# tamask1s/rspt

Hardware: AMD Instinct MI355X
Metric: MSamples/s compress (xdelta_hzr, 64ch x 65536 int32) (higher is better)
Workload: dtype int32

## Files before the change

rspt_amd/csrc/common.hpp:

```cpp
#pragma once
#include <hip/hip_runtime.h>
#include <stdint.h>

#ifdef RSPT_DIAG
#define RSPT_DIAG_ONLY(x) (x)
#else
#define RSPT_DIAG_ONLY(x) 0u
#endif

namespace rspt {

constexpr uint32_t kHzrBlock = 65536;
constexpr int kNumSym = 261;
constexpr uint32_t kRunCap = 16662;
constexpr int kSymStride = 264;
constexpr int kTdescWords = 92;
constexpr int kWave = 64;
constexpr int kEncThreads = 1024;
constexpr int kEncWaves = kEncThreads / kWave;
constexpr int kMaxPlanes = 4;
constexpr uint32_t kKindBytes = 4;

enum : uint32_t { kModeCopy = 0, kModeHuff = 1, kModeFill = 2, kModeSkip = 3, kModeStaged = 4 };

constexpr uint32_t kStageSlotWords = 772;

struct Geom {
    uint32_t bps, nch, ns;
    uint32_t N;
    uint32_t nblk;
    uint32_t hdr_len;
    uint32_t method;
    uint32_t kind;
    uint32_t be;
    uint64_t plane_stride;
// ... 240 lines not shown
```

rspt_amd/csrc/host_budget.hip:

```cpp
static size_t budget_tab_bytes(size_t nblocks, size_t nladder) { return (nladder * nblocks * sizeof(uint64_t) + 255) & ~(size_t)255; }

static bool budget_batched_ok(const rspt_hip_packer* p, size_t nblocks, size_t nladder) {
    const Geom& g = p->g;
    return g.kind == RSPT_HIP_KIND_HADAMARD && g.ns <= kTpMaxNs && nladder * nblocks <= 65535;
}

static int budget_route(const rspt_hip_packer* p, size_t nblocks, size_t nladder) {
    const bool ok = budget_batched_ok(p, nblocks, nladder);
    if (p->budget_route == 2) return ok ? 1 : RSPT_HIP_ERR_UNSUPPORTED;
    return p->budget_route == 0 && ok ? 1 : 0;
}

int rspt_hip_debug_set_budget_route(rspt_hip_packer* p, int route) {
    if (!p || route < 0 || route > 2) return RSPT_HIP_ERR_ARG;
    if (route == 2 && !budget_batched_ok(p, 1, 1)) return RSPT_HIP_ERR_UNSUPPORTED;
    p->budget_route = (uint32_t)route;
    return RSPT_HIP_OK;
}

int rspt_hip_compress_budget_work_bytes(rspt_hip_packer* p, size_t nblocks, size_t nladder, size_t* bytes) {
    if (!bytes) return RSPT_HIP_ERR_ARG;
    if (int rc = target_checks(p, nblocks, nladder)) return rc;
    if (int r = budget_route(p, nblocks, nladder); r < 0) return r;
    *bytes = budget_tab_bytes(nblocks, nladder);
// ... 24 lines not shown
}

static int budget_sizes_batched(rspt_hip_packer* p, const void* d_src, size_t nblocks, const LadderSel& ls, unsigned long long* tab,
                                hipStream_t st) {
    const Geom& g = p->g;
    const uint32_t B = (uint32_t)nblocks, S = ls.fwd.n * B;
    if (int rc = rspt_hip_reserve(p, S)) return rc;
    if (int rc = front_begin(p, S, st)) return rc;
    int32_t* orig = p->ws.planar + (size_t)(S - B) * g.N;
    if (int rc = rspt_hip_native_to_i32_batch_dev(p, d_src, orig, nblocks, (void*)st)) return rc;
    const uint32_t nt = std::max(64u, std::min(1024u, g.ns / kTpPer));
    const uint32_t lds = tp_pad(g.ns) * (uint32_t)sizeof(uint32_t);
    hipLaunchKernelGGL(k_budget_probe, dim3(g.nch, B), dim3(nt), lds, st, (const int32_t*)orig, g, ls.fwd, B, (int32_t*)p->ws.planar);
    hipLaunchKernelGGL((k_planar_planes<false>), dim3((g.N + 4095) / 4096, S), dim3(256), 0, st, p->ws.planar, g, (uint32_t)p->nb_host, p->ws.planes,
                       p->nzflag, (uint32_t*)nullptr);
    hipLaunchKernelGGL(k_nb_scan, dim3(1), dim3(1024), 0, st, p->needmask, S, p->nb_state, p->ws.nbuse, 0);
    const uint32_t nhb = S * kMaxPlanes * g.nblk;
    hipLaunchKernelGGL(k_histlist, dim3((nhb + 255) / 256), dim3(256), 0, st, p->nzflag, p->ws.nbuse, g, nhb, p->ws.big_list, p->work_ctr + 2, p->psel);
    HIPCHK(p, hipGetLastError());
    if (int rc = phase_hist(p, S, st)) return rc;
    if (int rc = phase_tree(p, S, st)) return rc;
    return budget_pass_end(p, S, tab, st);
}

int rspt_hip_compress_budget_batch_dev(rspt_hip_packer* p, const void* d_src, size_t nblocks, const double* ladder, size_t nladder,
                                       size_t budget_bytes, const uint64_t* d_budget, void* d_dst, size_t dst_stride, uint64_t* d_sizes,
                                       uint32_t* d_choice, uint64_t* d_cand_sizes, void* d_work, void* stream) {
    static_assert(sizeof(size_t) == sizeof(uint64_t), "budget_bytes carries any uint64");
    if (!p || !d_src || !d_dst || !d_sizes || !d_choice || !d_work || nblocks == 0) return RSPT_HIP_ERR_ARG;
    if ((reinterpret_cast<uintptr_t>(d_src) & 15) || (reinterpret_cast<uintptr_t>(d_choice) & 3) || (reinterpret_cast<uintptr_t>(d_budget) & 7) ||
        (reinterpret_cast<uintptr_t>(d_cand_sizes) & 7) || (reinterpret_cast<uintptr_t>(d_work) & 15))
        return RSPT_HIP_ERR_ARG;
    if (p->feed) return RSPT_HIP_ERR_ARG;
// ... 18 lines not shown
```

rspt_amd/csrc/host_handle.hpp:

```cpp
#pragma once

namespace {
enum Stage { ST_PRE = 0, ST_NB, ST_HIST, ST_TREE, ST_LAYOUT, ST_ENCODE, ST_COUNT };
const char* kStageNames[ST_COUNT] = {"preprocess", "nb_scan", "hzr_hist", "hzr_tree", "layout", "hzr_encode"};
}

template <class T, auto Release>
class Owned {
  public:
    Owned() = default;
    Owned(Owned&& o) noexcept : h_(o.h_) { o.h_ = nullptr; }
    Owned& operator=(Owned&& o) noexcept {
        if (this != &o) {
            reset();
            h_ = o.h_;
            o.h_ = nullptr;
        }
        return *this;
    }
    ~Owned() { reset(); }
    void reset() {
        if (h_) Release(h_);
        h_ = nullptr;
    }
// ... 7 lines not shown
    T h_ = nullptr;
};
template <class T> using Dev = Owned<T*, hipFree>;
template <class T> using Pinned = Owned<T*, hipHostFree>;
using Event = Owned<hipEvent_t, hipEventDestroy>;
using Stream = Owned<hipStream_t, hipStreamDestroy>;

struct Workspace {
    size_t cap_blocks = 0;
    size_t cap_slots = 0;
    Dev<uint8_t> planes;
    Dev<int32_t> planar;
    Dev<uint32_t> nbuse;
    Dev<uint32_t> dec_nb;
    Dev<uint32_t> big_list;
    Dev<uint32_t> staging;
    Dev<uint32_t> zbuf[2];
    size_t zcap_words = 0;
    bool zero_ready[2] = {false, false};
    int zset = 0;
    Dev<uint32_t> plane_dirty;
    bool planes_unknown = false;
    Dev<uint32_t> hist;
    Dev<uint32_t> seghist;
    Dev<uint32_t> segbase;
    Dev<uint32_t> lists;
    Dev<uint2> listinfo;
    Dev<uint32_t> cw;
    Dev<uint32_t> tdesc;
    Dev<BlockMeta> meta;
// ... 139 lines not shown
    double had_div_fwd = 0, had_div_inv = 0;
    bool dct_fft = false;
    uint32_t fft_l1 = 0, fft_l2 = 0;
    bool dct_real = false;
    uint32_t fftr_la = 0, fftr_lb = 0;
    uint32_t ntile = 0;
    uint32_t Tn_native = 0;
    uint32_t T = 0, in_lds = 0;
    uint32_t Tp[5] = {0, 0, 0, 0, 0};
    bool wide = false;
    uint32_t k1_threads = 256;
    uint32_t k1_grid = 0;
    uint32_t hist_grid = 0;
    uint32_t enc_grid = 0;
    uint32_t ablate = 0;
    uint32_t psel = 0;
    uint32_t target_route = 0;
    uint32_t budget_route = 0;
    uint32_t qp_form = 0;
    int verify = 0;
    int big_endian = 0;
    bool profiling = false;
    bool ev_valid = false;
    bool conv_lds_raised = false;

    Stream stream;
    Event ev[ST_COUNT + 1];
    Dev<unsigned long long> stamps;
    Dev<CrcConsts> crc;
    Dev<uint32_t> nb_state;
// ... 48 lines not shown
```

rspt_amd/csrc/hzr_kernels.hip:

```cpp
#include "common.hpp"

namespace rspt {

__device__ __forceinline__ uint32_t thread_id() {
    uint32_t t = threadIdx.x;
    asm volatile("" : "+v"(t));
    return t;
}

__device__ __forceinline__ uint32_t granule_byte_dyn(uint32_t w0, uint32_t w1, uint32_t w2, uint32_t w3, uint32_t i) {
    const uint32_t lo = (i & 8u) ? w2 : w0, hi = (i & 8u) ? w3 : w1;
    return __builtin_amdgcn_perm(hi, lo, 0x0C0C0C00u | (i & 7u));
}

constexpr uint32_t kWipeTokens = 2048;
__device__ __forceinline__ bool block_is_wiped(const BlockMeta& m) {
    return m.mode == kModeStaged || (m.mode == kModeHuff && m.fill <= kWipeTokens);
}
constexpr uint32_t kSmallSegments = 2;
constexpr uint32_t kSmallTokens = 512;
constexpr uint32_t kSmallPayload = 3072;
static_assert(kStageSlotWords * 4 >= 7 + kSmallPayload + 4 + 4, "staging slot too small");

struct WorkQueues {
    uint32_t n_big;
    uint32_t next_big;
};

struct WorkItem {
    uint32_t b, k, j;
};
__device__ __forceinline__ bool next_work(uint32_t* counter, uint32_t total, const Geom& g, uint32_t* s_slot, WorkItem& wi, uint32_t pass) {
    __syncthreads();
    if (threadIdx.x == 0) *s_slot = pass == 0 ? blockIdx.x : gridDim.x + atomicAdd(counter, 1u);
// ... 941 lines not shown
```

rspt_amd/csrc/planar.hip:

```cpp
#include "common.hpp"

namespace rspt {

constexpr uint32_t kPlanarThreads = 256;

__device__ __forceinline__ uint32_t cut_to_width(uint32_t v, uint32_t sx) { return (uint32_t)((int32_t)(v << sx) >> sx); }

template <bool XDELTA>
__global__ __launch_bounds__(kPlanarThreads) void k_planar_stream(const int32_t* __restrict__ src, Geom g, uint32_t kfirst, uint32_t kcount,
                                                                 uint8_t* __restrict__ planes, uint32_t* __restrict__ needmask,
                                                                 uint32_t* __restrict__ nzflag, const uint32_t* __restrict__ nbuse, uint32_t nblocks,
                                                                 uint32_t* __restrict__ ticket, uint32_t* __restrict__ nb_state,
                                                                 uint32_t* __restrict__ nbuse_out, const uint32_t* __restrict__ plane_dirty,
                                                                 uint32_t dirty_shift) {
    const uint32_t tid = threadIdx.x, l = lane_id();
    const bool fixup = nbuse != nullptr;
    if (fixup && *nb_state <= kfirst) return;
    const uint32_t sx = 32u - 8u * g.bps;
    const uint32_t segs = (g.N + 4095u) >> 12;
    const uint64_t total = (uint64_t)nblocks * segs;
    const uint64_t per = (total + gridDim.x - 1) / gridDim.x;
    const uint64_t w0 = (uint64_t)blockIdx.x * per, w1 = w0 + per < total ? w0 + per : total;
    uint32_t sent_b = 0xFFFFFFFFu, sent_f = 0;
    for (uint64_t w = w0; w < w1; ++w) {
        const uint32_t b = (uint32_t)(w / segs), seg = (uint32_t)(w - (uint64_t)b * segs);
        if (fixup && nbuse[b] <= kfirst) continue;
        const uint32_t off = (seg << 12) + tid * 16u;
        const uint32_t cnt = off < g.N ? min(16u, g.N - off) : 0u;
        const int32_t* pb = src + (size_t)b * g.N;
// ... 69 lines not shown
            if ((f & ~sent_f) && l == 0) atomicOr(&needmask[b], f);
            sent_f |= f;
        }
    }
    if (ticket) {
        __shared__ uint32_t s_last, s_wmax[16];
        __syncthreads();
        if (tid == 0) {
            __threadfence();
            s_last = atomicAdd(ticket, 1u) == gridDim.x - 1 ? 1u : 0u;
        }
        __syncthreads();
        if (s_last) {
            __threadfence();
            nb_scan_body(needmask, nblocks, nb_state, nbuse_out, XDELTA ? 1 : 0, s_wmax);
        }
    }
}
template __global__ void k_planar_stream<true>(const int32_t*, Geom, uint32_t, uint32_t, uint8_t*, uint32_t*, uint32_t*, const uint32_t*, uint32_t, uint32_t*, uint32_t*, uint32_t*, const uint32_t*, uint32_t);
template __global__ void k_planar_stream<false>(const int32_t*, Geom, uint32_t, uint32_t, uint8_t*, uint32_t*, uint32_t*, const uint32_t*, uint32_t, uint32_t*, uint32_t*, uint32_t*, const uint32_t*, uint32_t);

__global__ __launch_bounds__(256) void k_planar_ingest(const int32_t* __restrict__ src, Geom g, int32_t* __restrict__ planar,
                                                      long long* __restrict__ row_sum) {
    const uint32_t c = blockIdx.y, b = blockIdx.z, tid = threadIdx.x;
    const uint32_t sx = 32u - 8u * g.bps;
    const size_t base = (size_t)b * g.N + (size_t)c * g.ns;
    const uint32_t t0 = blockIdx.x * 4096u, t1 = min(g.ns, t0 + 4096u);
    long long sm = 0;
    for (uint32_t t = t0 + tid; t < t1; t += 256u) {
        const int32_t v = (int32_t)cut_to_width((uint32_t)src[base + t], sx);
        planar[base + t] = v;
        sm += v;
    }
    if (row_sum) {
#pragma unroll
// ... 20 lines not shown
```

rspt_amd/csrc/preprocess.hip:

```cpp
#include "common.hpp"

namespace rspt {

__device__ __forceinline__ uint32_t magic_of(uint32_t d) { return (uint32_t)(((1ull << 32) + d - 1) / d); }
__device__ __forceinline__ uint32_t fast_div(uint32_t q, uint32_t d, uint32_t M) { return d == 1 ? q : __umulhi(q, M); }

template <int BPS>
__device__ __forceinline__ int32_t sample_from_bytes(const uint8_t* p, bool aligned, bool be = false) {
    if (be) {
        if (BPS == 4) {
            if (aligned) {
                const uint32_t u = *reinterpret_cast<const uint32_t*>(p);
                return (int32_t)__builtin_amdgcn_perm(u, u, 0x00010203u);
            }
            return (int32_t)((uint32_t)p[3] | ((uint32_t)p[2] << 8) | ((uint32_t)p[1] << 16) | ((uint32_t)p[0] << 24));
        } else if (BPS == 3) {
            const uint32_t u = (uint32_t)p[2] | ((uint32_t)p[1] << 8) | ((uint32_t)p[0] << 16);
            return (int32_t)(u << 8) >> 8;
        } else if (BPS == 2) {
            const uint32_t u = (uint32_t)p[1] | ((uint32_t)p[0] << 8);
            return (int32_t)(u << 16) >> 16;
        }
        return (int32_t)(int8_t)p[0];
    }
// ... 35 lines not shown
    for (uint32_t b = lo; b < hi; ++b) m = max(m, need(b));
    const uint32_t l = lane_id(), w = tid >> 6;
    const uint32_t v = wave_scan_incl(m, 0u, [](uint32_t a, uint32_t c) { return a > c ? a : c; });
    if (l == 63) wmax[w] = v;
    __syncthreads();
    uint32_t pre = carry_in;
    for (uint32_t i = 0; i < w; ++i) pre = max(pre, wmax[i]);
    const uint32_t excl = dpp<0x138>(0u, v);
    uint32_t run = max(pre, l ? excl : 0u);
    for (uint32_t b = lo; b < hi; ++b) {
        run = max(run, need(b));
        nbuse[b] = run;
    }
    __syncthreads();
    if (tid == nthr - 1) *nb_state = max(pre, v);
}

struct ItemRegs {
    uint32_t pv[16];
    uint32_t p1, p2;
};

template <int BPS, bool XDELTA>
__device__ __forceinline__ void load_item(const uint8_t* blk, const Geom& g, uint32_t m_nch, uint32_t s0, uint32_t Tn, bool aligned4,
                                          uint32_t q, ItemRegs& R) {
    const size_t rstride = (size_t)g.nch * BPS;
    const uint32_t grp = fast_div(q, g.nch, m_nch);
    const uint32_t c = q - grp * g.nch;
    const uint32_t t0 = grp << 4;
    const uint32_t cnt = min(16u, Tn - t0);
// ... 131 lines not shown
#pragma unroll
            for (uint32_t k = 0; k < 4; ++k) {
                if (!((need >> k) & 1u)) continue;
                if (!(atomicOr(&za[k * g.nch], ba) & ba)) atomicOr(&nzflag[hb_index(g, b, k, ja)], ba);
                if (two && !(atomicOr(&zz[k * g.nch], bz) & bz)) atomicOr(&nzflag[hb_index(g, b, k, jz)], bz);
            }
        }
    }
}

template <int BPS, bool XDELTA>
__global__ __launch_bounds__(1024) void k_tile_planes(const uint8_t* __restrict__ src, Geom g, uint32_t T, uint32_t kfirst, uint32_t kcount,
                                                     uint8_t* __restrict__ planes, uint32_t* __restrict__ needmask,
                                                     uint32_t* __restrict__ nzflag, const uint32_t* __restrict__ nbuse, uint32_t ablate,
                                                     uint32_t nblocks, uint32_t* __restrict__ ticket, uint32_t* __restrict__ nb_state,
                                                     uint32_t* __restrict__ nbuse_out) {
    extern __shared__ __attribute__((aligned(16))) uint8_t lds[];
    const uint32_t tid = threadIdx.x, nthr = blockDim.x;
    const bool fixup = nbuse != nullptr;
    if (fixup && *nb_state <= kfirst) return;
    const uint32_t tiles_per_block = (g.ns + T - 1) / T;
    const uint32_t total = tiles_per_block * nblocks;
    const uint32_t m_nch = magic_of(g.nch);
    auto skip_untouched = [&](uint32_t wk) {
        while (wk < total && fixup && nbuse[wk / tiles_per_block] <= kfirst) wk += gridDim.x;
        return wk;
    };
    auto tile_s0 = [&](uint32_t wk) { return (wk - (wk / tiles_per_block) * tiles_per_block) * T; };
    uint32_t work = skip_untouched(blockIdx.x);
    ItemRegs cur, nxt, nx2;
    if (work < total) {
        const uint32_t s0f = tile_s0(work), Tnf = min(T, g.ns - s0f);
        const uint8_t* blkf = src + (size_t)(work / tiles_per_block) * g.block_bytes;
        if (tid < g.nch * ((Tnf + 15) >> 4))
// ... 69 lines not shown
        }
    }
    work = work_next;
    }
    if (ticket) {
        __shared__ uint32_t s_last, s_wmax[16];
        __syncthreads();
        if (tid == 0) {
            __threadfence();
            s_last = atomicAdd(ticket, 1u) == gridDim.x - 1 ? 1u : 0u;
        }
        __syncthreads();
        if (s_last) {
            __threadfence();
            nb_scan_body(needmask, nblocks, nb_state, nbuse_out, XDELTA ? 1 : 0, s_wmax);
        }
    }
}

template <int BPS>
__device__ __forceinline__ uint32_t stream_load(const uint8_t* base, uint32_t off) {
    uint32_t v;
    if (BPS == 1)
        asm volatile("global_load_sbyte %0, %1, %2" : "=v"(v) : "v"(off), "s"(base));
    else if (BPS == 2)
        asm volatile("global_load_sshort %0, %1, %2" : "=v"(v) : "v"(off), "s"(base));
    else
        asm volatile("global_load_dword %0, %1, %2" : "=v"(v) : "v"(off), "s"(base));
    return v;
}
// ... 501 lines not shown
        const uint32_t qpr = Tn >> 2;
        const uint32_t step_c = 256u / qpr, step_t = 256u - step_c * qpr;
        uint32_t c = tid / qpr, t4 = tid - c * qpr;
        for (uint32_t u = tid; u < g.nch * qpr; u += 256) {
            const int32_t* r = tile + c * RS + 4u * t4;
            *reinterpret_cast<int4*>(planar + (size_t)b * g.N + (size_t)c * g.ns + s0 + 4u * t4) = make_int4(r[0], r[1], r[2], r[3]);
            t4 += step_t;
            const uint32_t carry = t4 >= qpr ? 1u : 0u;
            t4 -= carry ? qpr : 0u;
            c += step_c + carry;
        }
    }
}

__global__ __launch_bounds__(1024) void k_nb_scan(const uint32_t* __restrict__ needmask, uint32_t nblocks, uint32_t* __restrict__ nb_state,
                                                  uint32_t* __restrict__ nbuse, int use_mask) {
    __shared__ uint32_t wmax[16];
    nb_scan_body(needmask, nblocks, nb_state, nbuse, use_mask, wmax);
}

#define INST_TILE(BPS)                                                                                                   \
    template __global__ void k_tile_planes<BPS, true>(const uint8_t*, Geom, uint32_t, uint32_t, uint32_t, uint8_t*, uint32_t*, uint32_t*, const uint32_t*, uint32_t, uint32_t, uint32_t*, uint32_t*, uint32_t*);    \
    template __global__ void k_tile_planes<BPS, false>(const uint8_t*, Geom, uint32_t, uint32_t, uint32_t, uint8_t*, uint32_t*, uint32_t*, const uint32_t*, uint32_t, uint32_t, uint32_t*, uint32_t*, uint32_t*);   \
    template __global__ void k_tile_planar<BPS>(const uint8_t*, Geom, uint32_t, int32_t*);
INST_TILE(1)
INST_TILE(2)
INST_TILE(3)
INST_TILE(4)
template __global__ void k_tile_stream<1, true, false>(const uint8_t*, Geom, uint32_t, uint32_t, uint32_t, uint8_t*, uint32_t*, uint32_t*, const uint32_t*, uint32_t, uint32_t, uint32_t*, uint32_t*, uint32_t*, const uint32_t*, uint32_t);
template __global__ void k_tile_stream<1, true, true>(const uint8_t*, Geom, uint32_t, uint32_t, uint32_t, uint8_t*, uint32_t*, uint32_t*, const uint32_t*, uint32_t, uint32_t, uint32_t*, uint32_t*, uint32_t*, const uint32_t*, uint32_t);
template __global__ void k_tile_stream<1, false, false>(const uint8_t*, Geom, uint32_t, uint32_t, uint32_t, uint8_t*, uint32_t*, uint32_t*, const uint32_t*, uint32_t, uint32_t, uint32_t*, uint32_t*, uint32_t*, const uint32_t*, uint32_t);
template __global__ void k_tile_stream<1, false, true>(const uint8_t*, Geom, uint32_t, uint32_t, uint32_t, uint8_t*, uint32_t*, uint32_t*, const uint32_t*, uint32_t, uint32_t, uint32_t*, uint32_t*, uint32_t*, const uint32_t*, uint32_t);
template __global__ void k_tile_stream<2, true, false>(const uint8_t*, Geom, uint32_t, uint32_t, uint32_t, uint8_t*, uint32_t*, uint32_t*, const uint32_t*, uint32_t, uint32_t, uint32_t*, uint32_t*, uint32_t*, const uint32_t*, uint32_t);
template __global__ void k_tile_stream<3, true, false>(const uint8_t*, Geom, uint32_t, uint32_t, uint32_t, uint8_t*, uint32_t*, uint32_t*, const uint32_t*, uint32_t, uint32_t, uint32_t*, uint32_t*, uint32_t*, const uint32_t*, uint32_t);
template __global__ void k_tile_stream<4, true, false>(const uint8_t*, Geom, uint32_t, uint32_t, uint32_t, uint8_t*, uint32_t*, uint32_t*, const uint32_t*, uint32_t, uint32_t, uint32_t*, uint32_t*, uint32_t*, const uint32_t*, uint32_t);
template __global__ void k_tile_stream<2, true, true>(const uint8_t*, Geom, uint32_t, uint32_t, uint32_t, uint8_t*, uint32_t*, uint32_t*, const uint32_t*, uint32_t, uint32_t, uint32_t*, uint32_t*, uint32_t*, const uint32_t*, uint32_t);
template __global__ void k_tile_stream<3, true, true>(const uint8_t*, Geom, uint32_t, uint32_t, uint32_t, uint8_t*, uint32_t*, uint32_t*, const uint32_t*, uint32_t, uint32_t, uint32_t*, uint32_t*, uint32_t*, const uint32_t*, uint32_t);
template __global__ void k_tile_stream<4, true, true>(const uint8_t*, Geom, uint32_t, uint32_t, uint32_t, uint8_t*, uint32_t*, uint32_t*, const uint32_t*, uint32_t, uint32_t, uint32_t*, uint32_t*, uint32_t*, const uint32_t*, uint32_t);
// ... 11 lines not shown
```

rspt_amd/csrc/rspt_hip.hip:

```cpp
#include "../../include/rspt_hip.h"

#include <hip/hip_runtime.h>
#include <dlfcn.h>
#include <link.h>
#include <climits>
#include <string>

#include <cmath>
#include <cstdio>
#include <cstdlib>
#include <cstring>
#include <memory>
#include <new>
#include <thread>
#include <type_traits>
#include <utility>
#include <vector>

#include "common.hpp"

#include "preprocess.hip"
#include "hzr_kernels.hip"
#include "hzr_rows.hip"
#include "transforms.hip"
// ... 94 lines not shown
    return T4 > g.ns ? g.ns : T4;
}

template <int BPS, bool XD>
static void launch_planes(rspt_hip_packer* p, const uint8_t* d_src, size_t nblocks, uint32_t kfirst, uint32_t kcount, const uint32_t* nbuse,
                          hipStream_t st) {
    const Geom& g = p->g;
    const uint32_t T = p->Tp[kcount];
    const bool stream_ok = (reinterpret_cast<uintptr_t>(d_src) & 3u) == 0 && g.ns >= 16 && g.block_bytes < (1ull << 32) && !(p->ablate & (1u << 22));
    const uint32_t lds = kcount * g.nch * (T + 16u) + 32u * g.nch + 96u;
    const uint32_t ntiles = (uint32_t)((g.ns + T - 1) / T * nblocks);
    const uint32_t per_cu = lds <= 40 * 1024 ? 4u : lds <= 80 * 1024 ? 2u : 1u;
    uint32_t want = per_cu * (uint32_t)p->num_cu;
    if (p->k1_grid) want = p->k1_grid;
    dim3 grid(want < ntiles ? want : ntiles);
    const bool stream = stream_ok;
    if (stream) {
        constexpr int SB = BPS;
        auto go = [&](auto kern) {
            hipFuncSetAttribute(reinterpret_cast<const void*>(kern), hipFuncAttributeMaxDynamicSharedMemorySize, (int)lds);
            hipLaunchKernelGGL(kern, grid, dim3(256), lds, st, d_src, g, T, kfirst, kcount, p->ws.planes, p->needmask, p->nzflag, nbuse, p->ablate,
                               (uint32_t)nblocks, nbuse ? nullptr : p->work_ctr + 1, p->nb_state, p->ws.nbuse, p->ws.plane_dirty, p->dirty_shift);
        };
        if (g.ns & 15u)
            go(&k_tile_stream<SB, XD, true>);
        else
            go(&k_tile_stream<SB, XD, false>);
        return;
    }
    hipFuncSetAttribute(reinterpret_cast<const void*>(&k_tile_planes<BPS, XD>), hipFuncAttributeMaxDynamicSharedMemorySize, (int)lds);
    hipLaunchKernelGGL((k_tile_planes<BPS, XD>), grid, dim3(p->k1_threads), lds, st, d_src, g, T, kfirst, kcount, p->ws.planes, p->needmask, p->nzflag, nbuse, p->ablate, (uint32_t)nblocks,
                       nbuse ? nullptr : p->work_ctr + 1, p->nb_state, p->ws.nbuse);
}

template <int BPS>
static uint32_t launch_front(rspt_hip_packer* p, const uint8_t* d_src, size_t nblocks, hipStream_t st) {
    const Geom& g = p->g;
    if (p->wide) {
        hipLaunchKernelGGL(k_wide_planar<BPS>, dim3((g.ns + 63) / 64, (g.nch + 63) / 64, (unsigned)nblocks), dim3(256), 0, st, d_src, g, p->ws.planar);
        if (g.kind == RSPT_HIP_KIND_XDELTA_HZR || g.kind == RSPT_HIP_KIND_HZR) {
            const bool xd = g.kind == RSPT_HIP_KIND_XDELTA_HZR;
            const dim3 pg((g.N + 4095) / 4096, (unsigned)nblocks);
            if (xd)
                hipLaunchKernelGGL((k_planar_planes<true>), pg, dim3(256), 0, st, p->ws.planar, g, 4u, p->ws.planes, p->nzflag, p->needmask);
            else
                hipLaunchKernelGGL((k_planar_planes<false>), pg, dim3(256), 0, st, p->ws.planar, g, 4u, p->ws.planes, p->nzflag, (uint32_t*)nullptr);
            hipLaunchKernelGGL(k_nb_scan, dim3(1), dim3(1024), 0, st, p->needmask, (uint32_t)nblocks, p->nb_state, p->ws.nbuse, xd ? 1 : 0);
        }
        return 4;
    }
    if (g.kind == RSPT_HIP_KIND_XDELTA_HZR) {
        const uint32_t np = p->nb_host;
        launch_planes<BPS, true>(p, d_src, nblocks, 0, np, nullptr, st);
        return np;
    }
    if (g.kind == RSPT_HIP_KIND_HZR) {
        launch_planes<BPS, false>(p, d_src, nblocks, 0, 4, nullptr, st);
        return 4;
    }
    if (BPS == 4 && (g.nch & 3) == 0 && (g.ns & 3) == 0 && g.nch <= 1024 && (reinterpret_cast<uintptr_t>(d_src) & 15) == 0) {
        const uint32_t T4 = tile_i32x4(g);
        hipLaunchKernelGGL(k_tile_planar_i32x4, dim3((g.ns + T4 - 1) / T4, (unsigned)nblocks), dim3(256), g.nch * (T4 + 1) * 4, st, d_src, g, T4,
// ... 3 lines not shown
    }
    dim3 grid((g.ns + p->T - 1) / p->T, (unsigned)nblocks);
    hipFuncSetAttribute(reinterpret_cast<const void*>(&k_tile_planar<BPS>), hipFuncAttributeMaxDynamicSharedMemorySize, (int)p->in_lds);
    hipLaunchKernelGGL((k_tile_planar<BPS>), grid, dim3(256), p->in_lds, st, d_src, g, p->T, p->ws.planar);
    return 4;
}

template <bool XD>
static void launch_planar_stream(rspt_hip_packer* p, const int32_t* d_planar, size_t nblocks, uint32_t kfirst, uint32_t kcount, const uint32_t* nbuse,
                                 hipStream_t st) {
    const Geom& g = p->g;
    const uint64_t units = (uint64_t)nblocks * ((g.N + 4095u) >> 12);
    const uint64_t want = 8ull * (uint64_t)p->num_cu;
    hipLaunchKernelGGL(k_planar_stream<XD>, dim3((uint32_t)(units < want ? units : want)), dim3(kPlanarThreads), 0, st, d_planar, g, kfirst, kcount, p->ws.planes,
                       p->needmask, p->nzflag, nbuse, (uint32_t)nblocks, nbuse ? nullptr : p->work_ctr + 1, p->nb_state, p->ws.nbuse, p->ws.plane_dirty,
                       p->dirty_shift);
}

static uint32_t launch_front_planar(rspt_hip_packer* p, const int32_t* d_planar, size_t nblocks, hipStream_t st) {
    const Geom& g = p->g;
    if (g.kind == RSPT_HIP_KIND_XDELTA_HZR) {
        const uint32_t np = p->nb_host;
        launch_planar_stream<true>(p, d_planar, nblocks, 0, np, nullptr, st);
        return np;
    }
    if (g.kind == RSPT_HIP_KIND_HZR) {
        launch_planar_stream<false>(p, d_planar, nblocks, 0, 4, nullptr, st);
        return 4;
    }
    hipLaunchKernelGGL(k_planar_ingest, dim3((g.ns + 4095u) / 4096u, g.nch, (unsigned)nblocks), dim3(256), 0, st, d_planar, g, p->ws.planar, p->row_sum);
    p->have_row_sum = p->row_sum != nullptr;
// ... 404 lines not shown
    HIPCHK(p, hipStreamSynchronize(p->stream));
    p->ws = Workspace();
    const Geom& g = p->g;
    Workspace w;
    const bool bare = g.kind == RSPT_HIP_KIND_BYTES;
    const size_t slots = slots_of(p, max_blocks);
    const size_t nhb = slots * kMaxPlanes * g.nblk;
    bool ok = true;
    ok &= hipMalloc(w.planes.out(), slots * kMaxPlanes * g.plane_stride + 4096) == hipSuccess;
    ok &= hipMalloc(w.nbuse.out(), max_blocks * sizeof(uint32_t)) == hipSuccess;
    ok &= hipMalloc(w.dec_nb.out(), max_blocks * sizeof(uint32_t)) == hipSuccess;
    ok &= hipMalloc(w.plane_dirty.out(), slots * kMaxPlanes * 4 * sizeof(uint32_t)) == hipSuccess;
    w.zcap_words = nhb + max_blocks + 32 + 2 * max_blocks * (size_t)g.nch + 2;
    for (int i = 0; i < 2; ++i) ok &= hipMalloc(w.zbuf[i].out(), w.zcap_words * sizeof(uint32_t)) == hipSuccess;
    ok &= hipMalloc(w.big_list.out(), nhb * sizeof(uint32_t)) == hipSuccess;
    ok &= hipMalloc(w.staging.out(), nhb * (size_t)kStageSlotWords * sizeof(uint32_t)) == hipSuccess;
    ok &= hipMalloc(w.hist.out(), nhb * kSymStride * sizeof(uint32_t)) == hipSuccess;
    ok &= hipMalloc(w.cw.out(), nhb * kSymStride * sizeof(uint32_t)) == hipSuccess;
    ok &= hipMalloc(w.seghist.out(), nhb * (size_t)kSegHistStride * sizeof(uint16_t)) == hipSuccess;
    ok &= hipMalloc(w.segbase.out(), nhb * (size_t)kEncWaves * sizeof(uint32_t)) == hipSuccess;
    ok &= hipMalloc(w.lists.out(), nhb * (size_t)kEncWaves * kListCap * sizeof(uint32_t)) == hipSuccess;
    ok &= hipMalloc(w.listinfo.out(), nhb * (size_t)kEncWaves * sizeof(uint2)) == hipSuccess;
    ok &= hipMalloc(w.tdesc.out(), nhb * kTdescWords * sizeof(uint32_t)) == hipSuccess;
    ok &= hipMalloc(w.meta.out(), nhb * sizeof(BlockMeta)) == hipSuccess;
    ok &= hipMalloc(w.out_off.out(), nhb * sizeof(uint64_t)) == hipSuccess;
    ok &= hipMalloc(w.means.out(), max_blocks * (size_t)(g.hdr_len ? g.hdr_len : 4)) == hipSuccess;
    if (!bare) ok &= hipMalloc(w.planar.out(), max_blocks * (size_t)g.N * sizeof(int32_t) + 4096) == hipSuccess;
    const size_t nscan = std::max<size_t>(p->ntile, g.N / kRowTile + 1);
    if (!bare) ok &= hipMalloc(w.txor.out(), max_blocks * nscan * sizeof(uint32_t)) == hipSuccess;
    if (!bare) ok &= hipMalloc(w.tsum.out(), max_blocks * nscan * sizeof(uint32_t)) == hipSuccess;
// ... 77 lines not shown
                               p->cos_tab, p->dct_scale0, p->dct_scale1, p->dct_cs0, p->ws.planar2);
        }
        hipLaunchKernelGGL((k_planar_planes<true>), dim3((g.N + 4095) / 4096, B), dim3(256), 0, st, p->ws.planar2, g, lossy_nb, p->ws.planes, nzflag, (uint32_t*)nullptr);
    }
}

static int front_begin(rspt_hip_packer* p, size_t nblocks, hipStream_t st) {
    const Geom& g = p->g;
    const size_t nhb_call = slots_of(p, nblocks) * kMaxPlanes * g.nblk;
    p->nzflag = p->ws.zbuf[p->ws.zset];
    p->needmask = p->nzflag + nhb_call;
    p->work_ctr = p->needmask + ((nblocks + 3) & ~(size_t)3);
    size_t zwords = (size_t)((p->work_ctr + 16) - p->nzflag);
    p->row_sum = nullptr;
    p->have_row_sum = false;
    if (g.kind == RSPT_HIP_KIND_DCT && p->dct_fft) {
        zwords = (zwords + 1) & ~(size_t)1;
        p->row_sum = reinterpret_cast<long long*>(p->nzflag + zwords);
        zwords += 2 * nblocks * (size_t)g.nch;
    }
    if (!p->ws.zero_ready[p->ws.zset]) HIPCHK(p, hipMemsetAsync(p->nzflag, 0, zwords * sizeof(uint32_t), st));
    p->ws.zero_ready[0] = p->ws.zero_ready[1] = false;
    if (p->ws.planes_unknown || (p->ablate & ~(3u << 26)) || p->psel) {
        HIPCHK(p, hipMemsetAsync(p->ws.plane_dirty, 0xFF, p->ws.cap_slots * kMaxPlanes * 4 * sizeof(uint32_t), st));
        p->ws.planes_unknown = false;
    }
    return RSPT_HIP_OK;
}

static int phase_front(rspt_hip_packer* p, const uint8_t* src, size_t nblocks, hipStream_t st, const int32_t* d_planar = nullptr, const LadderSel* ls = nullptr) {
    const Geom& g = p->g;
    const uint32_t B = (uint32_t)nblocks;
    stamp(p, ST_PRE, st);
    const bool xd = g.kind == RSPT_HIP_KIND_XDELTA_HZR;
    if (int rc = front_begin(p, nblocks, st)) return rc;
    if (g.kind == RSPT_HIP_KIND_BYTES) {
        const uint64_t units = (uint64_t)nblocks * ((g.N + 4095u) >> 12);
        const uint64_t want = 8ull * (uint64_t)p->num_cu;
        hipLaunchKernelGGL(k_bytes_ingest, dim3((uint32_t)(units < want ? units : want)), dim3(kIngestThreads), 0, st, src, g, B, p->ws.planes, p->nzflag,
                           p->ws.nbuse, p->ws.plane_dirty, p->dirty_shift);
        HIPCHK(p, hipGetLastError());
        stamp(p, ST_NB, st);
        stamp(p, ST_HIST, st);
        const uint32_t nhb = (uint32_t)slots_of(p, nblocks) * kMaxPlanes * g.nblk;
        hipLaunchKernelGGL(k_histlist, dim3((nhb + 255) / 256), dim3(256), 0, st, p->nzflag, p->ws.nbuse, g, nhb, p->ws.big_list, p->work_ctr + 2, p->psel);
        HIPCHK(p, hipGetLastError());
        return RSPT_HIP_OK;
    }
    const uint32_t np = d_planar ? launch_front_planar(p, d_planar, nblocks, st)
                                 : by_bps(g.bps, [&](auto bps) { return launch_front<decltype(bps)::value>(p, src, nblocks, st); });
    launch_forward_transform(p, B, st, p->nzflag, ls);
    HIPCHK(p, hipGetLastError());

    stamp(p, ST_NB, st);
    if (g.kind != RSPT_HIP_KIND_XDELTA_HZR && g.kind != RSPT_HIP_KIND_HZR)
        hipLaunchKernelGGL(k_nb_scan, dim3(1), dim3(1024), 0, st, p->needmask, B, p->nb_state, p->ws.nbuse, 0);
    if (xd && np < 4) {
        if (d_planar)
            launch_planar_stream<true>(p, d_planar, nblocks, np, 4 - np, p->ws.nbuse, st);
        else
            by_bps(g.bps, [&](auto bps) { launch_fixup<decltype(bps)::value>(p, src, nblocks, np, st); });
    }
    stamp(p, ST_HIST, st);
    const uint32_t nhb = B * kMaxPlanes * g.nblk;
    hipLaunchKernelGGL(k_histlist, dim3((nhb + 255) / 256), dim3(256), 0, st, p->nzflag, p->ws.nbuse, g, nhb, p->ws.big_list, p->work_ctr + 2, p->psel);
    HIPCHK(p, hipGetLastError());
    return RSPT_HIP_OK;
}

static uint32_t persistent_grid(const rspt_hip_packer* p, uint32_t nhb, uint32_t knob) {
    const uint32_t persist = (uint32_t)(2 * p->num_cu) < nhb ? (uint32_t)(2 * p->num_cu) : nhb;
    return knob && knob < persist ? knob : persist;
}

static int phase_hist(rspt_hip_packer* p, uint32_t B, hipStream_t st) {
    const Geom& g = p->g;
    const uint32_t nhb = B * kMaxPlanes * g.nblk;
    hipLaunchKernelGGL(k_hist, dim3(persistent_grid(p, nhb, p->hist_grid)), dim3(kEncThreads), 0, st, p->ws.planes, g, p->nzflag, p->ws.hist, p->ws.seghist, p->work_ctr,
                       p->ws.big_list, p->work_ctr + 2, p->ws.lists, p->ws.listinfo);
    HIPCHK(p, hipGetLastError());
    return RSPT_HIP_OK;
}

static int phase_tree(rspt_hip_packer* p, uint32_t B, hipStream_t st) {
    const Geom& g = p->g;
    const uint32_t nhb = B * kMaxPlanes * g.nblk;
    hipLaunchKernelGGL(k_tree, dim3((nhb + 3) / 4), dim3(256), 0, st, p->ws.hist, p->ws.planes, g, p->ws.nbuse, p->nzflag, nhb, p->ws.cw, p->ws.tdesc, p->ws.meta, p->ws.seghist, p->ws.segbase,
                       p->ws.zbuf[p->ws.zset ^ 1], (uint32_t)p->ws.zcap_words, p->crc, p->ws.staging, p->psel);
    HIPCHK(p, hipGetLastError());
    return RSPT_HIP_OK;
}

static int phase_layout(rspt_hip_packer* p, uint32_t B, void* d_dst, size_t dst_stride, uint64_t* d_sizes, hipStream_t st) {
    const Geom& g = p->g;
// ... 573 lines not shown
    if (!p || !host_buf || p->ws.cap_blocks == 0) return RSPT_HIP_ERR_ARG;
    if (hipSetDevice(p->device) != hipSuccess || hipDeviceSynchronize() != hipSuccess) return RSPT_HIP_ERR_LAUNCH;
    const Geom& g = p->g;
    const size_t nhb = p->ws.cap_slots * kMaxPlanes * g.nblk;
    const void* src = nullptr;
    size_t n = 0;
    switch (which) {
        case 0: src = p->ws.planes; n = p->ws.cap_slots * kMaxPlanes * g.plane_stride; break;
        case 1: src = p->ws.planar; n = p->ws.cap_blocks * (size_t)g.N * 4; break;
        case 2: src = p->ws.planar2; n = p->ws.planar2 ? p->ws.cap_blocks * (size_t)g.N * 4 : 0; break;
        case 3: src = p->ws.hist; n = nhb * kSymStride * 4; break;
        case 4: src = p->ws.meta; n = nhb * sizeof(BlockMeta); break;
        case 5: src = p->ws.nbuse; n = p->ws.cap_blocks * 4; break;
        case 6: src = p->ws.means; n = p->ws.cap_blocks * (size_t)g.hdr_len; break;
        case 8: src = p->nzflag; n = nhb * 4; break;
        case 7: src = p->stamps; n = (512 * 16 * 8 + 2 * 16384) * sizeof(unsigned long long); break;
        default: return RSPT_HIP_ERR_ARG;
    }
    if (!src || n == 0) return 0;
    if (n > cap) n = cap;
    if (hipMemcpy(host_buf, src, n, hipMemcpyDeviceToHost) != hipSuccess) return RSPT_HIP_ERR_LAUNCH;
    return (long long)n;
}

int rspt_hip_set_profiling(rspt_hip_packer* p, int on) {
    if (!p) return RSPT_HIP_ERR_ARG;
    p->profiling = on != 0;
    p->ev_valid = false;
    return RSPT_HIP_OK;
}
// ... 25 lines not shown
```

Baseline: 321,400.

## Fuse hist work-list construction into nb_scan and front-end kernel tails

```diff
diff --git a/rspt_amd/csrc/common.hpp b/rspt_amd/csrc/common.hpp
--- a/rspt_amd/csrc/common.hpp
+++ b/rspt_amd/csrc/common.hpp
@@ -19,6 +19,7 @@
 constexpr int kEncThreads = 1024;
 constexpr int kEncWaves = kEncThreads / kWave;
 constexpr int kMaxPlanes = 4;
+constexpr uint32_t kSmallSegments = 2;
 constexpr uint32_t kKindBytes = 4;
 
 enum : uint32_t { kModeCopy = 0, kModeHuff = 1, kModeFill = 2, kModeSkip = 3, kModeStaged = 4 };
diff --git a/rspt_amd/csrc/host_budget.hip b/rspt_amd/csrc/host_budget.hip
--- a/rspt_amd/csrc/host_budget.hip
+++ b/rspt_amd/csrc/host_budget.hip
@@ -62,9 +62,7 @@
     hipLaunchKernelGGL(k_budget_probe, dim3(g.nch, B), dim3(nt), lds, st, (const int32_t*)orig, g, ls.fwd, B, (int32_t*)p->ws.planar);
     hipLaunchKernelGGL((k_planar_planes<false>), dim3((g.N + 4095) / 4096, S), dim3(256), 0, st, p->ws.planar, g, (uint32_t)p->nb_host, p->ws.planes,
                        p->nzflag, (uint32_t*)nullptr);
-    hipLaunchKernelGGL(k_nb_scan, dim3(1), dim3(1024), 0, st, p->needmask, S, p->nb_state, p->ws.nbuse, 0);
-    const uint32_t nhb = S * kMaxPlanes * g.nblk;
-    hipLaunchKernelGGL(k_histlist, dim3((nhb + 255) / 256), dim3(256), 0, st, p->nzflag, p->ws.nbuse, g, nhb, p->ws.big_list, p->work_ctr + 2, p->psel);
+    launch_nb_scan(p, S, 0, st);
     HIPCHK(p, hipGetLastError());
     if (int rc = phase_hist(p, S, st)) return rc;
     if (int rc = phase_tree(p, S, st)) return rc;
diff --git a/rspt_amd/csrc/host_handle.hpp b/rspt_amd/csrc/host_handle.hpp
--- a/rspt_amd/csrc/host_handle.hpp
+++ b/rspt_amd/csrc/host_handle.hpp
@@ -45,6 +45,7 @@
     Dev<uint32_t> nbuse;
     Dev<uint32_t> dec_nb;
     Dev<uint32_t> big_list;
+    Dev<uint32_t> hist_list;
     Dev<uint32_t> staging;
     Dev<uint32_t> zbuf[2];
     size_t zcap_words = 0;
@@ -214,6 +215,7 @@
     uint32_t hist_grid = 0;
     uint32_t enc_grid = 0;
     uint32_t ablate = 0;
+    bool list_built = false;
     uint32_t psel = 0;
     uint32_t target_route = 0;
     uint32_t budget_route = 0;
diff --git a/rspt_amd/csrc/hzr_kernels.hip b/rspt_amd/csrc/hzr_kernels.hip
--- a/rspt_amd/csrc/hzr_kernels.hip
+++ b/rspt_amd/csrc/hzr_kernels.hip
@@ -17,7 +17,6 @@
 __device__ __forceinline__ bool block_is_wiped(const BlockMeta& m) {
     return m.mode == kModeStaged || (m.mode == kModeHuff && m.fill <= kWipeTokens);
 }
-constexpr uint32_t kSmallSegments = 2;
 constexpr uint32_t kSmallTokens = 512;
 constexpr uint32_t kSmallPayload = 3072;
 static_assert(kStageSlotWords * 4 >= 7 + kSmallPayload + 4 + 4, "staging slot too small");
diff --git a/rspt_amd/csrc/planar.hip b/rspt_amd/csrc/planar.hip
--- a/rspt_amd/csrc/planar.hip
+++ b/rspt_amd/csrc/planar.hip
@@ -12,7 +12,7 @@
                                                                  uint32_t* __restrict__ nzflag, const uint32_t* __restrict__ nbuse, uint32_t nblocks,
                                                                  uint32_t* __restrict__ ticket, uint32_t* __restrict__ nb_state,
                                                                  uint32_t* __restrict__ nbuse_out, const uint32_t* __restrict__ plane_dirty,
-                                                                 uint32_t dirty_shift) {
+                                                                 uint32_t dirty_shift, uint32_t* __restrict__ hist_list, uint32_t psel) {
     const uint32_t tid = threadIdx.x, l = lane_id();
     const bool fixup = nbuse != nullptr;
     if (fixup && *nb_state <= kfirst) return;
@@ -112,11 +112,12 @@
         if (s_last) {
             __threadfence();
             nb_scan_body(needmask, nblocks, nb_state, nbuse_out, XDELTA ? 1 : 0, s_wmax);
+            histlist_body(nzflag, nbuse_out, g.nblk, nblocks * kMaxPlanes * g.nblk, hist_list, ticket + 1, psel, s_wmax);
         }
     }
 }
-template __global__ void k_planar_stream<true>(const int32_t*, Geom, uint32_t, uint32_t, uint8_t*, uint32_t*, uint32_t*, const uint32_t*, uint32_t, uint32_t*, uint32_t*, uint32_t*, const uint32_t*, uint32_t);
-template __global__ void k_planar_stream<false>(const int32_t*, Geom, uint32_t, uint32_t, uint8_t*, uint32_t*, uint32_t*, const uint32_t*, uint32_t, uint32_t*, uint32_t*, uint32_t*, const uint32_t*, uint32_t);
+template __global__ void k_planar_stream<true>(const int32_t*, Geom, uint32_t, uint32_t, uint8_t*, uint32_t*, uint32_t*, const uint32_t*, uint32_t, uint32_t*, uint32_t*, uint32_t*, const uint32_t*, uint32_t, uint32_t*, uint32_t);
+template __global__ void k_planar_stream<false>(const int32_t*, Geom, uint32_t, uint32_t, uint8_t*, uint32_t*, uint32_t*, const uint32_t*, uint32_t, uint32_t*, uint32_t*, uint32_t*, const uint32_t*, uint32_t, uint32_t*, uint32_t);
 
 __global__ __launch_bounds__(256) void k_planar_ingest(const int32_t* __restrict__ src, Geom g, int32_t* __restrict__ planar,
                                                       long long* __restrict__ row_sum) {
diff --git a/rspt_amd/csrc/preprocess.hip b/rspt_amd/csrc/preprocess.hip
--- a/rspt_amd/csrc/preprocess.hip
+++ b/rspt_amd/csrc/preprocess.hip
@@ -73,6 +73,91 @@
     }
     __syncthreads();
     if (tid == nthr - 1) *nb_state = max(pre, v);
+}
+
+constexpr uint32_t kListBatch = 32;
+__device__ __forceinline__ void histlist_body(const uint32_t* __restrict__ nzflag, const uint32_t* __restrict__ nbuse, uint32_t nblk, uint32_t nhb_total,
+                                              uint32_t* __restrict__ list, uint32_t* __restrict__ count, uint32_t psel_arg, uint32_t* wsum) {
+    const uint32_t psel = RSPT_DIAG_ONLY(psel_arg);
+    const uint32_t tid = threadIdx.x, nthr = blockDim.x;
+    const uint32_t per = (nhb_total + nthr - 1) / nthr;
+    const uint32_t lo = min(nhb_total, tid * per), hi = min(nhb_total, lo + per);
+    __threadfence();
+    __syncthreads();
+    const uint32_t bj0 = lo / kMaxPlanes, b0 = bj0 / nblk;
+    struct Walk {
+        uint32_t k, j, b;
+    };
+    auto step = [&](Walk& w) {
+        if (++w.k == (uint32_t)kMaxPlanes) {
+            w.k = 0;
+            if (++w.j == nblk) {
+                w.j = 0;
+                ++w.b;
+            }
+        }
+    };
+    auto takes = [&](uint32_t v0, Walk& w) -> uint32_t {
+        uint32_t nz[kListBatch], nb[kListBatch];
+        Walk x = w;
+#pragma unroll
+        for (uint32_t i = 0; i < kListBatch; ++i) {
+            const Walk y = v0 + i < hi ? x : w;
+            nz[i] = __hip_atomic_load(&nzflag[(y.b * kMaxPlanes + y.k) * nblk + y.j], __ATOMIC_RELAXED, __HIP_MEMORY_SCOPE_AGENT);
+            nb[i] = __hip_atomic_load(&nbuse[y.b], __ATOMIC_RELAXED, __HIP_MEMORY_SCOPE_AGENT);
+            step(x);
+        }
+        uint32_t m = 0;
+        x = w;
+#pragma unroll
+        for (uint32_t i = 0; i < kListBatch; ++i) {
+            bool take = v0 + i < hi && x.k < nb[i] && (uint32_t)__popc(nz[i]) > kSmallSegments;
+            if (psel && ((x.k == 0 && (psel & 1u)) || (x.k >= 1 && (psel & 2u)))) take = false;
+            m |= (take ? 1u : 0u) << i;
+            step(x);
+        }
+        w = x;
+        return m;
+    };
+    const Walk w0{lo % kMaxPlanes, bj0 - b0 * nblk, b0};
+    uint32_t cnt = 0, m0 = 0, m1 = 0;
+    {
+        Walk w = w0;
+        for (uint32_t v0 = lo; v0 < hi; v0 += kListBatch) {
+            const uint32_t m = takes(v0, w);
+            if (v0 == lo) m0 = m;
+            if (v0 == lo + kListBatch) m1 = m;
+            cnt += (uint32_t)__popc(m);
+        }
+    }
+    const uint32_t incl = wave_scan_add(cnt);
+    if (lane_id() == 63) wsum[tid >> 6] = incl;
+    __syncthreads();
+    uint32_t pos = incl - cnt, total = 0;
+    for (uint32_t i = 0; i < (nthr >> 6); ++i) {
+        pos += i < (tid >> 6) ? wsum[i] : 0u;
+        total += wsum[i];
+    }
+    {
+        Walk w = w0;
+        for (uint32_t v0 = lo; v0 < hi; v0 += kListBatch) {
+            uint32_t m;
+            if (v0 == lo || v0 == lo + kListBatch) {
+                m = v0 == lo ? m0 : m1;
+            } else {
+                Walk r = w;
+                m = takes(v0, r);
+            }
+#pragma unroll
+            for (uint32_t i = 0; i < kListBatch; ++i) {
+                if ((m >> i) & 1u) list[pos++] = (w.b * kMaxPlanes + w.k) * nblk + w.j;
+                step(w);
+            }
+        }
+    }
+    __threadfence();
+    __syncthreads();
+    if (tid == 0) *count = total;
 }
 
 struct ItemRegs {
@@ -234,10 +319,15 @@
                                                      uint8_t* __restrict__ planes, uint32_t* __restrict__ needmask,
                                                      uint32_t* __restrict__ nzflag, const uint32_t* __restrict__ nbuse, uint32_t ablate,
                                                      uint32_t nblocks, uint32_t* __restrict__ ticket, uint32_t* __restrict__ nb_state,
-                                                     uint32_t* __restrict__ nbuse_out) {
+                                                     uint32_t* __restrict__ nbuse_out, uint32_t* __restrict__ hist_list,
+                                                     uint32_t* __restrict__ hist_count, uint32_t psel) {
     extern __shared__ __attribute__((aligned(16))) uint8_t lds[];
     const uint32_t tid = threadIdx.x, nthr = blockDim.x;
     const bool fixup = nbuse != nullptr;
+    if (fixup && hist_list && blockIdx.x == 0) {
+        __shared__ uint32_t s_wsum[16];
+        histlist_body(nzflag, nbuse, g.nblk, nblocks * kMaxPlanes * g.nblk, hist_list, hist_count, psel, s_wsum);
+    }
     if (fixup && *nb_state <= kfirst) return;
     const uint32_t tiles_per_block = (g.ns + T - 1) / T;
     const uint32_t total = tiles_per_block * nblocks;
@@ -337,6 +427,7 @@
         if (s_last) {
             __threadfence();
             nb_scan_body(needmask, nblocks, nb_state, nbuse_out, XDELTA ? 1 : 0, s_wmax);
+            if (hist_list) histlist_body(nzflag, nbuse_out, g.nblk, nblocks * kMaxPlanes * g.nblk, hist_list, ticket + 1, psel, s_wmax);
         }
     }
 }
@@ -868,14 +959,16 @@
 }
 
 __global__ __launch_bounds__(1024) void k_nb_scan(const uint32_t* __restrict__ needmask, uint32_t nblocks, uint32_t* __restrict__ nb_state,
-                                                  uint32_t* __restrict__ nbuse, int use_mask) {
+                                                  uint32_t* __restrict__ nbuse, int use_mask, const uint32_t* __restrict__ nzflag, uint32_t nblk,
+                                                  uint32_t* __restrict__ hist_list, uint32_t* __restrict__ hist_count, uint32_t psel) {
     __shared__ uint32_t wmax[16];
     nb_scan_body(needmask, nblocks, nb_state, nbuse, use_mask, wmax);
+    histlist_body(nzflag, nbuse, nblk, nblocks * kMaxPlanes * nblk, hist_list, hist_count, psel, wmax);
 }
 
 #define INST_TILE(BPS)                                                                                                   \
-    template __global__ void k_tile_planes<BPS, true>(const uint8_t*, Geom, uint32_t, uint32_t, uint32_t, uint8_t*, uint32_t*, uint32_t*, const uint32_t*, uint32_t, uint32_t, uint32_t*, uint32_t*, uint32_t*);    \
-    template __global__ void k_tile_planes<BPS, false>(const uint8_t*, Geom, uint32_t, uint32_t, uint32_t, uint8_t*, uint32_t*, uint32_t*, const uint32_t*, uint32_t, uint32_t, uint32_t*, uint32_t*, uint32_t*);   \
+    template __global__ void k_tile_planes<BPS, true>(const uint8_t*, Geom, uint32_t, uint32_t, uint32_t, uint8_t*, uint32_t*, uint32_t*, const uint32_t*, uint32_t, uint32_t, uint32_t*, uint32_t*, uint32_t*, uint32_t*, uint32_t*, uint32_t);   \
+    template __global__ void k_tile_planes<BPS, false>(const uint8_t*, Geom, uint32_t, uint32_t, uint32_t, uint8_t*, uint32_t*, uint32_t*, const uint32_t*, uint32_t, uint32_t, uint32_t*, uint32_t*, uint32_t*, uint32_t*, uint32_t*, uint32_t);  \
     template __global__ void k_tile_planar<BPS>(const uint8_t*, Geom, uint32_t, int32_t*);
 INST_TILE(1)
 INST_TILE(2)
diff --git a/rspt_amd/csrc/rspt_hip.hip b/rspt_amd/csrc/rspt_hip.hip
--- a/rspt_amd/csrc/rspt_hip.hip
+++ b/rspt_amd/csrc/rspt_hip.hip
@@ -132,7 +132,7 @@
     uint32_t want = per_cu * (uint32_t)p->num_cu;
     if (p->k1_grid) want = p->k1_grid;
     dim3 grid(want < ntiles ? want : ntiles);
-    const bool stream = stream_ok;
+    const bool stream = stream_ok && !nbuse;
     if (stream) {
         constexpr int SB = BPS;
         auto go = [&](auto kern) {
@@ -148,7 +148,22 @@
     }
     hipFuncSetAttribute(reinterpret_cast<const void*>(&k_tile_planes<BPS, XD>), hipFuncAttributeMaxDynamicSharedMemorySize, (int)lds);
     hipLaunchKernelGGL((k_tile_planes<BPS, XD>), grid, dim3(p->k1_threads), lds, st, d_src, g, T, kfirst, kcount, p->ws.planes, p->needmask, p->nzflag, nbuse, p->ablate, (uint32_t)nblocks,
-                       nbuse ? nullptr : p->work_ctr + 1, p->nb_state, p->ws.nbuse);
+                       nbuse ? nullptr : p->work_ctr + 1, p->nb_state, p->ws.nbuse, p->list_built ? nullptr : p->ws.hist_list, p->work_ctr + 2, p->psel);
+    p->list_built = true;
+}
+
+static size_t slots_of(const rspt_hip_packer* p, size_t nblocks);
+
+static void launch_histlist(rspt_hip_packer* p, size_t nblocks, hipStream_t st) {
+    const uint32_t nhb = (uint32_t)slots_of(p, nblocks) * kMaxPlanes * p->g.nblk;
+    hipLaunchKernelGGL(k_histlist, dim3((nhb + 255) / 256), dim3(256), 0, st, p->nzflag, p->ws.nbuse, p->g, nhb, p->ws.hist_list, p->work_ctr + 2, p->psel);
+    p->list_built = true;
+}
+
+static void launch_nb_scan(rspt_hip_packer* p, uint32_t nslots, int use_mask, hipStream_t st) {
+    hipLaunchKernelGGL(k_nb_scan, dim3(1), dim3(1024), 0, st, p->needmask, nslots, p->nb_state, p->ws.nbuse, use_mask, p->nzflag, p->g.nblk, p->ws.hist_list,
+                       p->work_ctr + 2, p->psel);
+    p->list_built = true;
 }
 
 template <int BPS>
@@ -163,7 +178,7 @@
                 hipLaunchKernelGGL((k_planar_planes<true>), pg, dim3(256), 0, st, p->ws.planar, g, 4u, p->ws.planes, p->nzflag, p->needmask);
             else
                 hipLaunchKernelGGL((k_planar_planes<false>), pg, dim3(256), 0, st, p->ws.planar, g, 4u, p->ws.planes, p->nzflag, (uint32_t*)nullptr);
-            hipLaunchKernelGGL(k_nb_scan, dim3(1), dim3(1024), 0, st, p->needmask, (uint32_t)nblocks, p->nb_state, p->ws.nbuse, xd ? 1 : 0);
+            launch_nb_scan(p, (uint32_t)nblocks, xd ? 1 : 0, st);
         }
         return 4;
     }
@@ -197,7 +212,8 @@
     const uint64_t want = 8ull * (uint64_t)p->num_cu;
     hipLaunchKernelGGL(k_planar_stream<XD>, dim3((uint32_t)(units < want ? units : want)), dim3(kPlanarThreads), 0, st, d_planar, g, kfirst, kcount, p->ws.planes,
                        p->needmask, p->nzflag, nbuse, (uint32_t)nblocks, nbuse ? nullptr : p->work_ctr + 1, p->nb_state, p->ws.nbuse, p->ws.plane_dirty,
-                       p->dirty_shift);
+                       p->dirty_shift, p->ws.hist_list, p->psel);
+    if (!nbuse) p->list_built = true;
 }
 
 static uint32_t launch_front_planar(rspt_hip_packer* p, const int32_t* d_planar, size_t nblocks, hipStream_t st) {
@@ -632,6 +648,7 @@
     w.zcap_words = nhb + max_blocks + 32 + 2 * max_blocks * (size_t)g.nch + 2;
     for (int i = 0; i < 2; ++i) ok &= hipMalloc(w.zbuf[i].out(), w.zcap_words * sizeof(uint32_t)) == hipSuccess;
     ok &= hipMalloc(w.big_list.out(), nhb * sizeof(uint32_t)) == hipSuccess;
+    ok &= hipMalloc(w.hist_list.out(), nhb * sizeof(uint32_t)) == hipSuccess;
     ok &= hipMalloc(w.staging.out(), nhb * (size_t)kStageSlotWords * sizeof(uint32_t)) == hipSuccess;
     ok &= hipMalloc(w.hist.out(), nhb * kSymStride * sizeof(uint32_t)) == hipSuccess;
     ok &= hipMalloc(w.cw.out(), nhb * kSymStride * sizeof(uint32_t)) == hipSuccess;
@@ -739,6 +756,7 @@
     size_t zwords = (size_t)((p->work_ctr + 16) - p->nzflag);
     p->row_sum = nullptr;
     p->have_row_sum = false;
+    p->list_built = false;
     if (g.kind == RSPT_HIP_KIND_DCT && p->dct_fft) {
         zwords = (zwords + 1) & ~(size_t)1;
         p->row_sum = reinterpret_cast<long long*>(p->nzflag + zwords);
@@ -767,8 +785,7 @@
         HIPCHK(p, hipGetLastError());
         stamp(p, ST_NB, st);
         stamp(p, ST_HIST, st);
-        const uint32_t nhb = (uint32_t)slots_of(p, nblocks) * kMaxPlanes * g.nblk;
-        hipLaunchKernelGGL(k_histlist, dim3((nhb + 255) / 256), dim3(256), 0, st, p->nzflag, p->ws.nbuse, g, nhb, p->ws.big_list, p->work_ctr + 2, p->psel);
+        launch_histlist(p, nblocks, st);
         HIPCHK(p, hipGetLastError());
         return RSPT_HIP_OK;
     }
@@ -779,7 +796,7 @@
 
     stamp(p, ST_NB, st);
     if (g.kind != RSPT_HIP_KIND_XDELTA_HZR && g.kind != RSPT_HIP_KIND_HZR)
-        hipLaunchKernelGGL(k_nb_scan, dim3(1), dim3(1024), 0, st, p->needmask, B, p->nb_state, p->ws.nbuse, 0);
+        launch_nb_scan(p, B, 0, st);
     if (xd && np < 4) {
         if (d_planar)
             launch_planar_stream<true>(p, d_planar, nblocks, np, 4 - np, p->ws.nbuse, st);
@@ -787,8 +804,7 @@
             by_bps(g.bps, [&](auto bps) { launch_fixup<decltype(bps)::value>(p, src, nblocks, np, st); });
     }
     stamp(p, ST_HIST, st);
-    const uint32_t nhb = B * kMaxPlanes * g.nblk;
-    hipLaunchKernelGGL(k_histlist, dim3((nhb + 255) / 256), dim3(256), 0, st, p->nzflag, p->ws.nbuse, g, nhb, p->ws.big_list, p->work_ctr + 2, p->psel);
+    if (!p->list_built) launch_histlist(p, nblocks, st);
     HIPCHK(p, hipGetLastError());
     return RSPT_HIP_OK;
 }
@@ -802,7 +818,7 @@
     const Geom& g = p->g;
     const uint32_t nhb = B * kMaxPlanes * g.nblk;
     hipLaunchKernelGGL(k_hist, dim3(persistent_grid(p, nhb, p->hist_grid)), dim3(kEncThreads), 0, st, p->ws.planes, g, p->nzflag, p->ws.hist, p->ws.seghist, p->work_ctr,
-                       p->ws.big_list, p->work_ctr + 2, p->ws.lists, p->ws.listinfo);
+                       p->ws.hist_list, p->work_ctr + 2, p->ws.lists, p->ws.listinfo);
     HIPCHK(p, hipGetLastError());
     return RSPT_HIP_OK;
 }
@@ -1406,6 +1422,8 @@
         case 5: src = p->ws.nbuse; n = p->ws.cap_blocks * 4; break;
         case 6: src = p->ws.means; n = p->ws.cap_blocks * (size_t)g.hdr_len; break;
         case 8: src = p->nzflag; n = nhb * 4; break;
+        case 9: src = p->ws.hist_list; n = nhb * 4; break;
+        case 10: src = p->work_ctr; n = 16 * 4; break;
         case 7: src = p->stamps; n = (512 * 16 * 8 + 2 * 16384) * sizeof(unsigned long long); break;
         default: return RSPT_HIP_ERR_ARG;
     }
```

Result: slower. 317,300 (-1.3%).
